# succinctlabs/sp1

Measured on NVIDIA H100. Metric: riscv_cycles_proven_per_second_core, higher is better.
Workload: dtype u32 KoalaBear (Montgomery) / ext4

## Files before the change

### sp1_b200/csrc/ntt.cu

```cuda
#include "ctx.cuh"
#include <cstdlib>
#include "kb31.cuh"
#include "sumcheck.cuh"

namespace {

__global__ void init_tables_kernel(uint32_t* TH, uint32_t* TL) {
    uint32_t i = blockIdx.x * blockDim.x + threadIdx.x;
    if (i >= 4096) return;
    uint32_t w = kb::pow(kb::to_monty_c(3), 127);
    TL[i] = kb::pow(w, i);
    TH[i] = kb::pow(w, (uint64_t)i << 12);
}

__global__ void rs_step_a_generic(const uint32_t* __restrict__ in, uint32_t* __restrict__ out, int L1, int L2, int b, int T,
                                  const uint32_t* __restrict__ TH, const uint32_t* __restrict__ TL) {
    extern __shared__ uint32_t sm[];
    const int L = L1 + L2;
    const size_t n = (size_t)1 << L, M = n << b;
    const uint32_t* col_in = in + (size_t)blockIdx.y * n;
    uint32_t* col_out = out + (size_t)blockIdx.y * M;
    const uint32_t lo0 = blockIdx.x * T;
    const int H = 1 << L1;
    const int tile = H * T;
    for (int r = 0; r < (1 << b); r++) {
        const uint32_t rr = __brev((uint32_t)r) >> (32 - b);
        for (int idx = threadIdx.x; idx < tile; idx += blockDim.x) {
            int hi = idx / T, lo = idx - hi * T;
            uint32_t x = col_in[((size_t)hi << L2) + lo0 + lo];
            if (r && hi) x = kb::mul(x, root_pow(TH, TL, ((uint32_t)hi * r) << (24 - L1 - b)));
            sm[idx] = x;
        }
        __syncthreads();
        for (int s = L1; s >= 1; s--) {
            const int half = 1 << (s - 1);
            for (int w = threadIdx.x; w < (H / 2) * T; w += blockDim.x) {
                int bf = w / T, lo = w - bf * T;
                int j = bf & (half - 1), blk = bf >> (s - 1);
                int i0 = ((blk << s) + j) * T + lo, i1 = i0 + half * T;
                uint32_t a = sm[i0], c = sm[i1];
                sm[i0] = kb::add(a, c);
                uint32_t d = kb::sub(a, c);
                sm[i1] = j ? kb::mul(d, __ldg(TH + ((uint32_t)j << (12 - s)))) : d;
            }
            __syncthreads();
        }
        for (int idx = threadIdx.x; idx < tile; idx += blockDim.x) {
            int p = idx / T, lo = idx - p * T;
            col_out[(((size_t)rr << L1) + p << L2) + lo0 + lo] = sm[idx];
        }
        __syncthreads();
    }
}

__global__ void rs_step_b_generic(uint32_t* __restrict__ buf, int L1, int L2, int b, const uint32_t* __restrict__ TH,
                                  const uint32_t* __restrict__ TL) {
    extern __shared__ uint32_t sm[];
    const int L = L1 + L2;
    const size_t M = (size_t)1 << (L + b);
    const uint32_t q = blockIdx.x;
    const uint32_t ka = (L1 + b) ? (__brev(q) >> (32 - (L1 + b))) : 0;
    uint32_t* row = buf + (size_t)blockIdx.y * M + ((size_t)q << L2);
    const int W = 1 << L2;
    for (int lo = threadIdx.x; lo < W; lo += blockDim.x) {
        uint32_t x = row[lo];
        uint32_t e = ((uint32_t)lo * ka) << (24 - L - b);
        if (e) x = kb::mul(x, root_pow(TH, TL, e));
        sm[lo] = x;
    }
    __syncthreads();
    for (int s = L2; s >= 1; s--) {
        const int half = 1 << (s - 1);
        for (int w = threadIdx.x; w < W / 2; w += blockDim.x) {
            int j = w & (half - 1), blk = w >> (s - 1);
            int i0 = (blk << s) + j, i1 = i0 + half;
            uint32_t a = sm[i0], c = sm[i1];
            sm[i0] = kb::add(a, c);
            uint32_t d = kb::sub(a, c);
            sm[i1] = j ? kb::mul(d, __ldg(TH + ((uint32_t)j << (12 - s)))) : d;
        }
        __syncthreads();
    }
    for (int lo = threadIdx.x; lo < W; lo += blockDim.x) row[lo] = sm[lo];
}


__device__ __forceinline__ uint32_t submul(uint32_t a, uint32_t c, uint32_t w) { return kb::mul(a - c + kb::P, w); }

__device__ __forceinline__ void dif8(uint32_t (&v)[8], const uint32_t (&wA)[4], const uint32_t (&wB)[2], uint32_t wC) {
#pragma unroll
    for (int j = 0; j < 4; j++) { uint32_t a = v[j], c = v[j + 4]; v[j] = kb::add(a, c); v[j + 4] = submul(a, c, wA[j]); }
#pragma unroll
    for (int h = 0; h < 8; h += 4)
#pragma unroll
        for (int j = 0; j < 2; j++) { uint32_t a = v[h + j], c = v[h + j + 2]; v[h + j] = kb::add(a, c); v[h + j + 2] = submul(a, c, wB[j]); }
#pragma unroll
    for (int h = 0; h < 8; h += 2) { uint32_t a = v[h], c = v[h + 1]; v[h] = kb::add(a, c); v[h + 1] = submul(a, c, wC); }
}

__device__ __forceinline__ void load_tw8(const uint32_t* __restrict__ TH, int s, uint32_t low, uint32_t (&wA)[4], uint32_t (&wB)[2],
                                         uint32_t& wC) {
    const uint32_t stride = 1u << (s - 3);
#pragma unroll
    for (int j = 0; j < 4; j++) wA[j] = __ldg(TH + ((j * stride + low) << (12 - s)));
#pragma unroll
    for (int j = 0; j < 2; j++) wB[j] = __ldg(TH + ((j * stride + low) << (13 - s)));
    wC = __ldg(TH + (low << (14 - s)));
}

__device__ __forceinline__ int swzB(int e) { return e ^ (((e >> 5) & 7) << 2); }

__global__ void __launch_bounds__(256) rs_step_b_2048(uint32_t* __restrict__ buf, int L1, int b, const uint32_t* __restrict__ TH,
                                                      const uint32_t* __restrict__ TL) {
    __shared__ uint32_t sm[2048];
    constexpr int L2 = 11;
    const int L = L1 + L2;
    const size_t M = (size_t)1 << (L + b);
    const uint32_t q = blockIdx.x;
    const uint32_t ka = (L1 + b) ? (__brev(q) >> (32 - (L1 + b))) : 0;
    uint32_t* row = buf + (size_t)blockIdx.y * M + ((size_t)q << L2);
    const int t = threadIdx.x;
    uint32_t v[8], wA[4], wB[2], wC;
#pragma unroll
    for (int j = 0; j < 8; j++) v[j] = row[j * 256 + t];
    if (ka) {
        const int sh = 24 - L - b;
        uint32_t tw = root_pow(TH, TL, ((uint32_t)t * ka) << sh);
        const uint32_t step = root_pow(TH, TL, ((256u * ka) << sh) & 0xffffffu);
#pragma unroll
        for (int j = 0; j < 8; j++) { v[j] = kb::mul(v[j], tw); if (j < 7) tw = kb::mul(tw, step); }
    }
    load_tw8(TH, 11, t, wA, wB, wC);
    dif8(v, wA, wB, wC);
#pragma unroll
    for (int j = 0; j < 8; j++) sm[swzB(j * 256 + t)] = v[j];
    __syncthreads();
    {
        const int low = t & 31, hib = t >> 5;
#pragma unroll
        for (int j = 0; j < 8; j++) v[j] = sm[swzB(hib * 256 + j * 32 + low)];
        load_tw8(TH, 8, low, wA, wB, wC);
        dif8(v, wA, wB, wC);
#pragma unroll
        for (int j = 0; j < 8; j++) sm[swzB(hib * 256 + j * 32 + low)] = v[j];
    }
    __syncthreads();
    {
        const int low = t & 3, hib = t >> 2;
#pragma unroll
        for (int j = 0; j < 8; j++) v[j] = sm[swzB(hib * 32 + j * 4 + low)];
        load_tw8(TH, 5, low, wA, wB, wC);
        dif8(v, wA, wB, wC);
#pragma unroll
        for (int j = 0; j < 8; j++) sm[swzB(hib * 32 + j * 4 + low)] = v[j];
    }
    __syncthreads();
    const uint32_t w4 = __ldg(TH + 1024);
#pragma unroll
    for (int k = 0; k < 2; k++) {
        const int g = t + k * 256;
        uint4 x = *reinterpret_cast<const uint4*>(&sm[swzB(4 * g)]);
        uint32_t a0 = kb::add(x.x, x.z), a1 = kb::add(x.y, x.w);
        uint32_t a2 = kb::sub(x.x, x.z), a3 = submul(x.y, x.w, w4);
        uint4 y = make_uint4(kb::add(a0, a1), kb::sub(a0, a1), kb::add(a2, a3), kb::sub(a2, a3));
        *reinterpret_cast<uint4*>(row + 4 * g) = y;
    }
}

__device__ __forceinline__ int swzA(int e) { return e ^ (((e >> 7) & 1) << 4); }

template <int L1, int MINB = 1>
__global__ void __launch_bounds__(1 << L1, MINB) rs_step_a_fast(const uint32_t* __restrict__ in, uint32_t* __restrict__ out, int L2, int b,
                                                          const uint32_t* __restrict__ TH, const uint32_t* __restrict__ TL) {
    static_assert(L1 % 3 == 1 && L1 >= 7, "L1 = 3k+1, at least two radix-8 passes");
    constexpr int NP = L1 / 3;
    constexpr int TILE = 8 << L1;
    extern __shared__ uint32_t smA[];
    const int L = L1 + L2;
    const size_t n = (size_t)1 << L, M = n << b;
    const uint32_t* col_in = in + (size_t)blockIdx.y * n;
    uint32_t* col_out = out + (size_t)blockIdx.y * M;
    const uint32_t lo0 = blockIdx.x * 8;
    const int u = threadIdx.x, lo = u & 7, x = u >> 3;
    uint32_t src[8], v[8], wA[4], wB[2], wC;
#pragma unroll
    for (int j = 0; j < 8; j++) src[j] = col_in[((size_t)(j * (1 << (L1 - 3)) + x) << L2) + lo0 + lo];
    const int sh = 24 - L1 - b;
    for (int r = 0; r < (1 << b); r++) {
        uint32_t* sm = smA + (r & 1) * TILE;
        const uint32_t rr = __brev((uint32_t)r) >> (32 - b);
        if (r == 0) {
#pragma unroll
            for (int j = 0; j < 8; j++) v[j] = src[j];
        } else {
            uint32_t tw = root_pow(TH, TL, ((uint32_t)x * r) << sh);
            const uint32_t step = root_pow(TH, TL, ((uint32_t)r << (L1 - 3)) << sh);
#pragma unroll
            for (int j = 0; j < 8; j++) { v[j] = kb::mul(src[j], tw); if (j < 7) tw = kb::mul(tw, step); }
        }
        load_tw8(TH, L1, x, wA, wB, wC);
        dif8(v, wA, wB, wC);
#pragma unroll
        for (int j = 0; j < 8; j++) sm[swzA(j * (TILE / 8) + u)] = v[j];
        __syncthreads();
#pragma unroll
        for (int k = 1; k < NP; k++) {
            const int hb = L1 - 1 - 3 * k;
            const int nlow = hb - 2;
            const int low = x & ((1 << nlow) - 1), high = x >> nlow;
            const int base = ((high << (hb + 1)) + low) * 8 + lo;
            const int stride = 8 << nlow;
#pragma unroll
            for (int j = 0; j < 8; j++) v[j] = sm[swzA(base + j * stride)];
            load_tw8(TH, hb + 1, low, wA, wB, wC);
            dif8(v, wA, wB, wC);
            if (k < NP - 1) {
#pragma unroll
                for (int j = 0; j < 8; j++) sm[swzA(base + j * stride)] = v[j];
                __syncthreads();
            } else {
                const bool odd = (x & 1);
#pragma unroll
                for (int j = 0; j < 8; j++) {
                    uint32_t o = __shfl_xor_sync(0xffffffffu, v[j], 8);
                    uint32_t res = odd ? kb::sub(o, v[j]) : kb::add(v[j], o);
                    const uint32_t p = (uint32_t)((high << 4) + j * 2 + (x & 1));
                    col_out[((((size_t)rr << L1) + p) << L2) + lo0 + lo] = res;
                }
            }
        }
    }
}

}

template <int L1, int MINB = 1>
static sp1b200_err launch_step_a_fast(sp1b200_ctx* ctx, const uint32_t* in, uint32_t* out, int L2, int b, unsigned nc) {
    const size_t smem = 2 * (size_t)(8 << L1) * sizeof(uint32_t);
    SP1_CUDA(cudaFuncSetAttribute(rs_step_a_fast<L1, MINB>, cudaFuncAttributeMaxDynamicSharedMemorySize, (int)smem));
    dim3 g((1u << L2) / 8, nc);
    SP1_LAUNCH(ctx, (rs_step_a_fast<L1, MINB>), g, 1 << L1, smem, in, out, L2, b, ctx->d_TH, ctx->d_TL);
    return nullptr;
}

sp1b200_err sp1b200_init_tables(sp1b200_ctx* ctx) {
    SP1_CUDA(cudaMalloc(&ctx->d_TH, 4096 * sizeof(uint32_t)));
    SP1_CUDA(cudaMalloc(&ctx->d_TL, 4096 * sizeof(uint32_t)));
    SP1_LAUNCH(ctx, init_tables_kernel, 16, 256, 0, ctx->d_TH, ctx->d_TL);
    return nullptr;
}

sp1b200_err sp1b200_rs_encode_device(sp1b200_ctx* ctx, const uint32_t* d_msg, uint64_t ncols, uint32_t log_h,
                                     uint32_t log_blowup, uint32_t* d_out) {
    if (log_blowup < 1 || log_blowup > 4) return sp1b200_set_error("rs_encode: log_blowup %u unsupported (1..4)", log_blowup);
    if (log_h + log_blowup > 24) return sp1b200_set_error("rs_encode: 2^%u exceeds the two-adicity 2^24", log_h + log_blowup);
    if (ncols == 0) return nullptr;
    const int L = (int)log_h, b = (int)log_blowup;
    const int L2 = L < 11 ? L : 11;
    const int L1 = L - L2;
    if (L1 > 12) return sp1b200_set_error("rs_encode: log_h %u too large", log_h);
    int T = 16;
    if ((1 << L2) < T) T = 1 << L2;
    while (((size_t)T << L1) * 4 > 160 * 1024) T >>= 1;
    const size_t smemA = ((size_t)T << L1) * sizeof(uint32_t);
    const size_t smemB = ((size_t)1 << L2) * sizeof(uint32_t);
    SP1_CUDA(cudaFuncSetAttribute(rs_step_a_generic, cudaFuncAttributeMaxDynamicSharedMemorySize, 200 * 1024));
    const size_t n = (size_t)1 << L, M = n << b;
    size_t group = (64ull << 20) / (M * sizeof(uint32_t));
    if (group < 1) group = 1;
    if (group > 65535) group = 65535;
    int threadsA = (int)(((size_t)T << L1) / 2);
    if (threadsA > 1024) threadsA = 1024;
    if (threadsA < 32) threadsA = 32;
    int threadsB = (1 << L2) / 2;
    if (threadsB > 1024) threadsB = 1024;
    if (threadsB < 32) threadsB = 32;
    const bool fast = (L2 == 11) && !ctx->force_generic_ntt;
    for (uint64_t c0 = 0; c0 < ncols; c0 += group) {
        unsigned nc = (unsigned)((ncols - c0 < group) ? (ncols - c0) : group);
        dim3 gA((1u << L2) / T, nc), gB(1u << (L1 + b), nc);
        static const bool occ2 = [] { const char* e = getenv("SP1B200_RS_A_OCC2"); return !(e && e[0] == '0'); }();
        if (fast && L1 == 10 && occ2) SP1_TRY((launch_step_a_fast<10, 2>(ctx, d_msg + c0 * n, d_out + c0 * M, L2, b, nc)));
        else if (fast && L1 == 10) SP1_TRY(launch_step_a_fast<10>(ctx, d_msg + c0 * n, d_out + c0 * M, L2, b, nc));
        else if (fast && L1 == 7) SP1_TRY(launch_step_a_fast<7>(ctx, d_msg + c0 * n, d_out + c0 * M, L2, b, nc));
        else SP1_LAUNCH(ctx, rs_step_a_generic, gA, threadsA, smemA, d_msg + c0 * n, d_out + c0 * M, L1, L2, b, T, ctx->d_TH, ctx->d_TL);
        if (fast) SP1_LAUNCH(ctx, rs_step_b_2048, gB, 256, 0, d_out + c0 * M, L1, b, ctx->d_TH, ctx->d_TL);
        else SP1_LAUNCH(ctx, rs_step_b_generic, gB, threadsB, smemB, d_out + c0 * M, L1, L2, b, ctx->d_TH, ctx->d_TL);
    }
    return nullptr;
}
```

Baseline: 55.42 million.

## Add coset-based LDE path for RS encode with row-persistent step B

Adds a new step-A kernel that splits the low-degree extension into 2^b cosets. It reads each message column once, multiplies by coset shift powers, and runs a size-2^L1 DIF per coset with twiddles folded into the output. A persistent row kernel then performs the 2048-point stage, double-buffering the next row in registers. Columns are no longer chunked into groups, and the old path stays reachable through an environment variable. This aims to remove the repeated reads and zero-padded work of the full-size transform, at the cost of extra multiplies and more register pressure.

```diff
diff --git a/sp1_b200/csrc/ntt.cu b/sp1_b200/csrc/ntt.cu
--- a/sp1_b200/csrc/ntt.cu
+++ b/sp1_b200/csrc/ntt.cu
@@ -232,6 +232,144 @@
     }
 }
 
+
+__device__ __forceinline__ int swzL(int e) { return e ^ (((e >> 6) & 3) << 3); }
+
+template <int L1, int MINB = (1024 >> L1)>
+__global__ void __launch_bounds__(1 << L1, MINB) rs_step_a_lde(const uint32_t* __restrict__ in, uint32_t* __restrict__ out, int b,
+                                                           const uint32_t* __restrict__ TH, const uint32_t* __restrict__ TL) {
+    static_assert(L1 % 3 != 2 && L1 >= 6, "L1 = 3k or 3k+1");
+    constexpr int L2 = 11, NP = L1 / 3, TILE = 8 << L1;
+    constexpr bool SHFL = L1 % 3 == 1;
+    extern __shared__ uint32_t smL[];
+    const size_t n = (size_t)1 << (L1 + L2);
+    const uint32_t* col_in = in + (size_t)blockIdx.y * n + blockIdx.x * 8;
+    uint32_t* col_out = out + ((size_t)blockIdx.y * n << b) + blockIdx.x * 8;
+    const int u = threadIdx.x, lo = u & 7, x = u >> 3;
+    uint32_t src[8], zh[8], v[8], wA[NP][4], wB[NP][2], wC[NP];
+#pragma unroll
+    for (int j = 0; j < 8; j++) src[j] = col_in[(size_t)((j << (L1 - 3)) + x) * (1 << L2) + lo];
+    load_tw8(TH, L1, x, wA[0], wB[0], wC[0]);
+#pragma unroll
+    for (int k = 1; k < NP; k++) {
+        const int hb = L1 - 1 - 3 * k;
+        load_tw8(TH, hb + 1, x & ((1 << (hb - 2)) - 1), wA[k], wB[k], wC[k]);
+    }
+    const uint32_t lg = blockIdx.x * 8 + lo;
+    {
+        const int sh = 24 - L1 - L2 - b;
+        const uint32_t step = root_pow(TH, TL, (1u << (L1 - 3 + L2)) << sh);
+        zh[0] = root_pow(TH, TL, (((uint32_t)x << L2) + lg) << sh);
+#pragma unroll
+        for (int j = 1; j < 8; j++) zh[j] = kb::mul(zh[j - 1], step);
+    }
+    uint32_t ft[8];
+#pragma unroll
+    for (int j = 0; j < 8; j++) {
+        const uint32_t p = SHFL ? ((x >> 1) << 4) + 2 * j + (x & 1) : (x << 3) + j;
+        ft[j] = root_pow(TH, TL, (lg * (__brev(p) >> (32 - L1))) << (24 - L1 - L2));
+    }
+    for (int r = 0; r < (1 << b); r++) {
+        uint32_t* sm = smL + (r & 1) * TILE;
+        uint32_t* row_out = col_out + ((size_t)(__brev((uint32_t)r) >> (32 - b)) << (L1 + L2));
+        if (r) {
+#pragma unroll
+            for (int j = 0; j < 8; j++) src[j] = kb::mul(src[j], zh[j]);
+        }
+#pragma unroll
+        for (int j = 0; j < 8; j++) v[j] = src[j];
+        dif8(v, wA[0], wB[0], wC[0]);
+#pragma unroll
+        for (int j = 0; j < 8; j++) sm[swzL(j * (TILE / 8) + u)] = v[j];
+        __syncthreads();
+#pragma unroll
+        for (int k = 1; k < NP; k++) {
+            const int hb = L1 - 1 - 3 * k;
+            const int nlow = hb - 2;
+            const int low = x & ((1 << nlow) - 1), high = x >> nlow;
+            const int base = ((high << (hb + 1)) + low) * 8 + lo;
+#pragma unroll
+            for (int j = 0; j < 8; j++) v[j] = sm[swzL(base + (j << (nlow + 3)))];
+            dif8(v, wA[k], wB[k], wC[k]);
+            if (k < NP - 1) {
+#pragma unroll
+                for (int j = 0; j < 8; j++) sm[swzL(base + (j << (nlow + 3)))] = v[j];
+                __syncthreads();
+            } else if (SHFL) {
+                const bool odd = (x & 1);
+#pragma unroll
+                for (int j = 0; j < 8; j++) {
+                    uint32_t o = __shfl_xor_sync(0xffffffffu, v[j], 8);
+                    row_out[(size_t)((high << 4) + j * 2 + (x & 1)) * (1 << L2) + lo] = kb::mul(odd ? kb::sub(o, v[j]) : kb::add(v[j], o), ft[j]);
+                }
+            } else {
+#pragma unroll
+                for (int j = 0; j < 8; j++) row_out[(size_t)((x << 3) + j) * (1 << L2) + lo] = kb::mul(v[j], ft[j]);
+            }
+        }
+    }
+}
+
+__global__ void __launch_bounds__(256, 4) rs_step_b_rows(uint32_t* __restrict__ buf, int lk, const uint32_t* __restrict__ TH) {
+    __shared__ uint32_t smR[2][2048];
+    constexpr int L2 = 11;
+    const uint32_t rows = 1u << lk;
+    uint32_t* col = buf + ((size_t)blockIdx.y << (L2 + lk));
+    const int t = threadIdx.x;
+    uint32_t w1A[4], w1B[2], w1C, w2A[4], w2B[2], w2C, w3A[4], w3B[2], w3C;
+    load_tw8(TH, 11, t, w1A, w1B, w1C);
+    load_tw8(TH, 8, t & 31, w2A, w2B, w2C);
+    load_tw8(TH, 5, t & 3, w3A, w3B, w3C);
+    const uint32_t w4 = __ldg(TH + 1024);
+    uint32_t nx[8];
+    uint32_t q = blockIdx.x;
+    if (q < rows) {
+#pragma unroll
+        for (int j = 0; j < 8; j++) nx[j] = col[((size_t)q << L2) + j * 256 + t];
+    }
+    for (int it = 0; q < rows; q += gridDim.x, it ^= 1) {
+        uint32_t* row = col + ((size_t)q << L2);
+        uint32_t* sm = smR[it];
+        uint32_t v[8];
+#pragma unroll
+        for (int j = 0; j < 8; j++) v[j] = nx[j];
+        if (q + gridDim.x < rows) {
+#pragma unroll
+            for (int j = 0; j < 8; j++) nx[j] = row[((size_t)gridDim.x << L2) + j * 256 + t];
+        }
+        dif8(v, w1A, w1B, w1C);
+#pragma unroll
+        for (int j = 0; j < 8; j++) sm[swzB(j * 256 + t)] = v[j];
+        __syncthreads();
+        {
+            const int low = t & 31, hib = t >> 5;
+#pragma unroll
+            for (int j = 0; j < 8; j++) v[j] = sm[swzB(hib * 256 + j * 32 + low)];
+            dif8(v, w2A, w2B, w2C);
+#pragma unroll
+            for (int j = 0; j < 8; j++) sm[swzB(hib * 256 + j * 32 + low)] = v[j];
+        }
+        __syncthreads();
+        {
+            const int low = t & 3, hib = t >> 2;
+#pragma unroll
+            for (int j = 0; j < 8; j++) v[j] = sm[swzB(hib * 32 + j * 4 + low)];
+            dif8(v, w3A, w3B, w3C);
+#pragma unroll
+            for (int j = 0; j < 8; j++) sm[swzB(hib * 32 + j * 4 + low)] = v[j];
+        }
+        __syncthreads();
+#pragma unroll
+        for (int k = 0; k < 2; k++) {
+            const int g = t + k * 256;
+            uint4 x = *reinterpret_cast<const uint4*>(&sm[swzB(4 * g)]);
+            uint32_t a0 = kb::add(x.x, x.z), a1 = kb::add(x.y, x.w);
+            uint32_t a2 = kb::sub(x.x, x.z), a3 = submul(x.y, x.w, w4);
+            *reinterpret_cast<uint4*>(row + 4 * g) = make_uint4(kb::add(a0, a1), kb::sub(a0, a1), kb::add(a2, a3), kb::sub(a2, a3));
+        }
+    }
+}
+
 }
 
 template <int L1, int MINB = 1>
@@ -240,6 +378,14 @@
     SP1_CUDA(cudaFuncSetAttribute(rs_step_a_fast<L1, MINB>, cudaFuncAttributeMaxDynamicSharedMemorySize, (int)smem));
     dim3 g((1u << L2) / 8, nc);
     SP1_LAUNCH(ctx, (rs_step_a_fast<L1, MINB>), g, 1 << L1, smem, in, out, L2, b, ctx->d_TH, ctx->d_TL);
+    return nullptr;
+}
+
+template <int L1, int MINB = (1024 >> L1)>
+static sp1b200_err launch_step_a_lde(sp1b200_ctx* ctx, const uint32_t* in, uint32_t* out, int b, unsigned nc) {
+    const size_t smem = 2 * (size_t)(8 << L1) * sizeof(uint32_t);
+    SP1_CUDA(cudaFuncSetAttribute(rs_step_a_lde<L1, MINB>, cudaFuncAttributeMaxDynamicSharedMemorySize, (int)smem));
+    SP1_LAUNCH(ctx, (rs_step_a_lde<L1, MINB>), dim3((1u << 11) / 8, nc), 1 << L1, smem, in, out, b, ctx->d_TH, ctx->d_TL);
     return nullptr;
 }
 
@@ -266,7 +412,10 @@
     const size_t smemB = ((size_t)1 << L2) * sizeof(uint32_t);
     SP1_CUDA(cudaFuncSetAttribute(rs_step_a_generic, cudaFuncAttributeMaxDynamicSharedMemorySize, 200 * 1024));
     const size_t n = (size_t)1 << L, M = n << b;
-    size_t group = (64ull << 20) / (M * sizeof(uint32_t));
+    const bool fast = (L2 == 11) && !ctx->force_generic_ntt;
+    const char* old_env = getenv("SP1B200_RS_OLD");
+    const bool lde = fast && !(old_env && old_env[0] == '1') && (L1 == 10 || L1 == 9 || L1 == 7);
+    size_t group = lde ? ncols : (64ull << 20) / (M * sizeof(uint32_t));
     if (group < 1) group = 1;
     if (group > 65535) group = 65535;
     int threadsA = (int)(((size_t)T << L1) / 2);
@@ -275,17 +424,25 @@
     int threadsB = (1 << L2) / 2;
     if (threadsB > 1024) threadsB = 1024;
     if (threadsB < 32) threadsB = 32;
-    const bool fast = (L2 == 11) && !ctx->force_generic_ntt;
+    const unsigned rows = 1u << (L1 + b);
     for (uint64_t c0 = 0; c0 < ncols; c0 += group) {
         unsigned nc = (unsigned)((ncols - c0 < group) ? (ncols - c0) : group);
-        dim3 gA((1u << L2) / T, nc), gB(1u << (L1 + b), nc);
-        static const bool occ2 = [] { const char* e = getenv("SP1B200_RS_A_OCC2"); return !(e && e[0] == '0'); }();
-        if (fast && L1 == 10 && occ2) SP1_TRY((launch_step_a_fast<10, 2>(ctx, d_msg + c0 * n, d_out + c0 * M, L2, b, nc)));
-        else if (fast && L1 == 10) SP1_TRY(launch_step_a_fast<10>(ctx, d_msg + c0 * n, d_out + c0 * M, L2, b, nc));
-        else if (fast && L1 == 7) SP1_TRY(launch_step_a_fast<7>(ctx, d_msg + c0 * n, d_out + c0 * M, L2, b, nc));
-        else SP1_LAUNCH(ctx, rs_step_a_generic, gA, threadsA, smemA, d_msg + c0 * n, d_out + c0 * M, L1, L2, b, T, ctx->d_TH, ctx->d_TL);
-        if (fast) SP1_LAUNCH(ctx, rs_step_b_2048, gB, 256, 0, d_out + c0 * M, L1, b, ctx->d_TH, ctx->d_TL);
-        else SP1_LAUNCH(ctx, rs_step_b_generic, gB, threadsB, smemB, d_out + c0 * M, L1, L2, b, ctx->d_TH, ctx->d_TL);
+        dim3 gA((1u << L2) / T, nc), gB(rows, nc);
+        const uint32_t* src = d_msg + c0 * n;
+        uint32_t* dst = d_out + c0 * M;
+        if (lde) {
+            if (L1 == 10) SP1_TRY(launch_step_a_lde<10>(ctx, src, dst, b, nc));
+            else if (L1 == 9) SP1_TRY(launch_step_a_lde<9>(ctx, src, dst, b, nc));
+            else SP1_TRY(launch_step_a_lde<7>(ctx, src, dst, b, nc));
+            const unsigned per_col = rows > 16 ? rows / 16 : 1;
+            SP1_LAUNCH(ctx, rs_step_b_rows, dim3(per_col, nc), 256, 0, dst, L1 + b, ctx->d_TH);
+            continue;
+        }
+        if (fast && L1 == 10) SP1_TRY((launch_step_a_fast<10, 2>(ctx, src, dst, L2, b, nc)));
+        else if (fast && L1 == 7) SP1_TRY(launch_step_a_fast<7>(ctx, src, dst, L2, b, nc));
+        else SP1_LAUNCH(ctx, rs_step_a_generic, gA, threadsA, smemA, src, dst, L1, L2, b, T, ctx->d_TH, ctx->d_TL);
+        if (fast) SP1_LAUNCH(ctx, rs_step_b_2048, gB, 256, 0, dst, L1, b, ctx->d_TH, ctx->d_TL);
+        else SP1_LAUNCH(ctx, rs_step_b_generic, gB, threadsB, smemB, dst, L1, L2, b, ctx->d_TH, ctx->d_TL);
     }
     return nullptr;
 }
```

After: 56.34 million, median of 6. +1.7%, better.
